# zmoon/crt1d

Measured on AMD Instinct MI355X. Metric: (column x band) solves/sec at 60 layers, higher is better.
Workload: dtype f64

## Files before the change

### crt1d_amd/_lib.py

```python

import ctypes
import os

_HERE = os.path.dirname(os.path.abspath(__file__))
LIB_PATH = os.environ.get("CRT1D_HIP_LIB") or os.path.join(_HERE, "libcrt1d_hip.so")

SCHEME_IDS = {"2s": 0, "4s": 1, "n79": 2, "zq": 3, "bl": 4, "g77": 5, "bf": 6, "zq_pa": 7}
F32_SCHEMES = ("2s", "4s", "n79", "zq", "bl", "g77", "bf", "zq_pa")
TAU_D_METHODS = {"quad": 0, "9sky": 1}
NQ_TAU, NQ_G4, NQ_9SKY = 96, 32, 9
NQ = NQ_TAU + NQ_G4 + NQ_9SKY

FLAG_SKIP_PRECOMPUTE = 1
FLAG_PRECOMPUTE_ONLY = 2
FLAG_DIRECT_STORES = 4

MAX_LEVEL_SELECT = 64

CRT_OK = 0
CRT_ERR_BAD_ARG = -1
CRT_ERR_WORKSPACE = -2
CRT_ERR_UNSUPPORTED = -3
CRT_ERR_LAUNCH = -4
CRT_ERR_SHAPE = -5

_vp = ctypes.c_void_p


class CrtColumns(ctypes.Structure):
    _fields_ = [
        ("ncol", ctypes.c_int32),
        ("nz", ctypes.c_int32),
        ("psi", _vp),
        ("lai", _vp),
        ("mla", _vp),
        ("g_kind", _vp),
        ("g_param", _vp),
        ("g_at_psi", _vp),
        ("g_table", _vp),
    ]


class CrtBands(ctypes.Structure):
    _fields_ = [
        ("nb", ctypes.c_int32),
        ("col_stride", ctypes.c_int64),
        ("I_dr0", _vp),
        ("I_df0", _vp),
        ("leaf_r", _vp),
        ("leaf_t", _vp),
        ("soil_r", _vp),
    ]


class CrtSunSeries(ctypes.Structure):

    _fields_ = [
        ("nt", ctypes.c_int32),
        ("psi", _vp),
        ("g_at_psi", _vp),
        ("col_stride", ctypes.c_int64),
        ("I_dr0", _vp),
        ("I_df0", _vp),
    ]


class CrtSunSeriesF32(CrtSunSeries):
    """crt_sun_series_f32: the layout of crt_sun_series with float I_dr0 / I_df0 behind the pointers (crt_hip_levels_series_f32)."""


NTUNE = 16

TUNE_TILE_LDS = 0
TUNE_TILE_T = 1
TUNE_TILE_FLAGS = 2
TUNE_CLOSED_STORE_WAVES = 3
TUNE_CLOSED_PIPE_T = 4
TUNE_PACK = 5
TUNE_PACK_COMPUTE_WAVES = 6
TUNE_TRI_M = 8
TUNE_TRI_T = 9
TUNE_TRI_FAMILY = 10
TUNE_TRI_STORE_WAVES = 11
TUNE_MIN_TILE_NB = 12
TUNE_FLAT_FLUSH = 13
TUNE_K0_SEPARATE = 15
TILE_FLAG_SYNC_BARRIERS = 1
TILE_FLAG_GENERIC_FLUSH = 2
TILE_FLAG_NO_PIPELINE = 4
TILE_FLAG_NO_GENERIC_PIPELINE = 8
TILE_FLAG_FOUR_PAIR_STORE = 16
PACK_OFF = 1
PACK_FORCE = 2
TRI_FAMILY_NO_PIPELINE = 1
TRI_FAMILY_DOUBLE_BUFFERED = 2
TRI_FAMILY_REG_STAGED = 3
TRI_FAMILY_GENERIC_PIPELINE = 4
TRI_FAMILY_ZQPA_TWO_KERNEL = 1
TRI_FAMILY_ZQPA_PIPE = 5
TRI_FAMILY_ZQPA_PIPE2_DB = 6
TRI_FAMILY_ZQPA_PIPE2_RS = 7
FLAT_FLUSH_OFF = 1
FLAT_FLUSH_PART_LINE = 2
FLAT_FLUSH_WHOLE_LINE = 3


class CrtOptions(ctypes.Structure):
    _fields_ = [("mu_s", ctypes.c_double), ("tau_d_method", ctypes.c_int32), ("flags", ctypes.c_int32), ("tune", ctypes.c_int32 * NTUNE)]


def set_tune(opts, tune):
    for k in tune:
        if not isinstance(k, int) or not 0 <= k < NTUNE:
            raise ValueError(f"unknown crt_options.tune key {k!r}: keys are the TUNE_* constants, 0 .. {NTUNE - 1}")
    for k in range(NTUNE):
        opts.tune[k] = int(tune.get(k, 0))
    return opts


class CrtOutputs(ctypes.Structure):
    _fields_ = [(k, _vp) for k in ("I_dr", "I_df_d", "I_df_u", "F", "x0", "x1", "x2")]


class CrtBandsumOut(ctypes.Structure):

    _fields_ = [(k, _vp) for k in ("aI", "aI_sl", "aI_sh", "totals", "aI_dr", "I_dr", "I_df_d", "I_df_u", "F", "I_d")]


ABI_VERSION = 3


def _signatures():
    P = ctypes.POINTER
    i, i32, i64, sz, dbl, ok = ctypes.c_int, ctypes.c_int32, ctypes.c_int64, ctypes.c_size_t, ctypes.c_double, ctypes.c_int
    cols, bands, opts, outs, sums = P(CrtColumns), P(CrtBands), P(CrtOptions), P(CrtOutputs), P(CrtBandsumOut)
    solve = [cols, bands, opts, outs, _vp, sz, _vp]
    t = {
        "crt_hip_abi_version": (i, None),
        "crt_hip_strerror": (ctypes.c_char_p, [i]),
        "crt_hip_workspace_bytes": (sz, [i, i32, i32]),
        "crt_hip_workspace_bytes_nb": (sz, [i, i32, i32, i32]),
        "crt_hip_series_workspace_bytes": (sz, [i, i32, i32, i32, i32]),
        "crt_hip_levels_series_workspace_bytes": (sz, [i, i32, i32, i32]),
        "crt_hip_quad_nodes": (ok, [dbl, P(dbl)]),
        "crt_hip_integrated_series_f64": (ok, [i, cols, bands, P(CrtSunSeries), opts, _vp, i32, sums, _vp, sz, _vp]),
    }
    for suffix, sun_t in (("f64", CrtSunSeries), ("f32", CrtSunSeriesF32)):
        t[f"crt_hip_solve_{suffix}"] = (ok, [i] + solve)
        for s in SCHEME_IDS if suffix == "f64" else F32_SCHEMES:
            t[f"crt_hip_{s}_{suffix}"] = (ok, solve)
        t[f"crt_hip_absorb_{suffix}"] = (ok, [cols, bands, _vp, _vp, _vp, P(_vp), _vp, _vp, _vp])
        t[f"crt_hip_absorb_bandsum_{suffix}"] = (ok, [cols, bands, _vp, _vp, _vp, _vp, i32, _vp, _vp, _vp, _vp, _vp])
        t[f"crt_hip_absorb_bandsum2_{suffix}"] = (ok, [cols, bands, _vp, _vp, _vp, _vp, i32, sums, _vp])
        t[f"crt_hip_integrated_{suffix}"] = (ok, [i, cols, bands, opts, _vp, i32, _vp, _vp, _vp, _vp, _vp, sz, _vp])
        t[f"crt_hip_integrated2_{suffix}"] = (ok, [i, cols, bands, opts, _vp, i32, sums, _vp, sz, _vp])
        t[f"crt_hip_levels_{suffix}"] = (ok, [i, cols, bands, opts, P(i32), i32, outs, _vp, sz, _vp])
        t[f"crt_hip_levels_series_{suffix}"] = (ok, [i, cols, bands, P(sun_t), opts, P(i32), i32, outs, _vp, sz, _vp])
    t.update({
        "crt_hip_bandsum_finish_f64": (ok, [cols, i32, sums, _vp]),
        "crt_hip_band_reduce_f64": (ok, [_vp, i64, i32, _vp, i32, _vp, _vp]),
        "crt_hip_tau_d_f64": (ok, [_vp, _vp, i64, i32, _vp, _vp]),
        "crt_hip_smear_tuv_f64": (ok, [_vp, i64, i32, _vp, i32, _vp, i32, _vp, _vp]),
        "crt_hip_lai_beta_f64": (ok, [_vp, _vp, _vp, i32, i32, _vp, _vp, _vp, _vp]),
        "crt_hip_buffer_alloc_set": (ok, [i32, P(sz), P(_vp)]),
        "crt_hip_buffer_alloc": (ok, [sz, P(_vp)]),
        "crt_hip_buffer_free": (ok, [_vp]),
        "crt_hip_buffer_trim": (ok, []),
        "crt_hip_buffer_set_retain": (ok, [sz]),
        "crt_hip_buffer_describe": (ok, [_vp, ctypes.c_char_p, sz]),
        "crt_hip_buffer_stats": (ok, [P(i64)]),
        "crt_hip_last_kernel": (ctypes.c_char_p, []),
        "crt_hip_probe_fill_f64": (ok, [_vp, sz, dbl, _vp]),
        "crt_hip_probe_copy_f64": (ok, [_vp, _vp, sz, _vp]),
        "crt_hip_probe_store_set_f64": (ok, [P(_vp), i32, i64, i64, i32, dbl, _vp]),
# ... 61 lines not shown
```

### crt1d_amd/csrc/crt_internal.hpp

```cpp
#pragma once
#include <hip/hip_runtime.h>
#include <stddef.h>
#include <stdint.h>

#include "crt1d_hip.h"

namespace crt {

enum RecScalar {
  S_KB = 0,
  S_MU = 1,
  S_G = 2,
  S_MUBAR = 3,
  S_GINT1 = 4,
  S_GINT2 = 5,
  S_DLM = 6,
  S_TAUI = 7,
  S_TPSI = 8,
  S_COS2 = 9,
  S_LT = 10,
  S_INVMU = 11,
  S_UNIF = 12,
  S_DL = 13,
  S_M = 14,
// ... 258 lines not shown
  double* aI_dr;
  double* L_dr;
  double* L_dn;
  double* L_up;
  double* L_F;
  double* L_Id;
};

template <int CTRL>
__device__ inline double dpp_add(double v) {
  const int lo = __builtin_amdgcn_update_dpp(0, __double2loint(v), CTRL, 0xf, 0xf, false);
  const int hi = __builtin_amdgcn_update_dpp(0, __double2hiint(v), CTRL, 0xf, 0xf, false);
  return v + __hiloint2double(hi, lo);
}
__device__ inline double row_sum16(double v) {
  v = dpp_add<0xB1>(v);
  v = dpp_add<0x4E>(v);
  v = dpp_add<0x141>(v);
  v = dpp_add<0x140>(v);
  return v;
}
template <int CTRL, int ROW_MASK>
__device__ inline double dpp_add_rows(double v) {
  const int lo = __builtin_amdgcn_update_dpp(0, __double2loint(v), CTRL, ROW_MASK, 0xf, false);
  const int hi = __builtin_amdgcn_update_dpp(0, __double2hiint(v), CTRL, ROW_MASK, 0xf, false);
  return v + __hiloint2double(hi, lo);
}
__device__ inline double wave_sum_lane63(double v) {
  v = row_sum16(v);
  v = dpp_add_rows<0x142, 0xA>(v);
  v = dpp_add_rows<0x143, 0xC>(v);
  return v;
}
__device__ inline double swap_add32(double x, double y) {
  const auto lo = __builtin_amdgcn_permlane32_swap(__double2loint(x), __double2loint(y), false, false);
  const auto hi = __builtin_amdgcn_permlane32_swap(__double2hiint(x), __double2hiint(y), false, false);
  return __hiloint2double(hi[0], lo[0]) + __hiloint2double(hi[1], lo[1]);
}
__device__ inline double swap_add16(double x, double y) {
  const auto lo = __builtin_amdgcn_permlane16_swap(__double2loint(x), __double2loint(y), false, false);
  const auto hi = __builtin_amdgcn_permlane16_swap(__double2hiint(x), __double2hiint(y), false, false);
  return __hiloint2double(hi[0], lo[0]) + __hiloint2double(hi[1], lo[1]);
}
__device__ inline double wave_sum4(double a, double b, double c, double d) {
  return row_sum16(swap_add16(swap_add32(a, b), swap_add32(c, d)));
}
__device__ inline int wave_sum4_slot(int row) { return ((row & 1) << 1) | (row >> 1); }
template <int N>
__device__ inline void wave_sum_store(const double (&v)[N], double* dst, int nvalid, int lane) {
  const int slot = wave_sum4_slot(lane >> 4);
#pragma unroll
  for (int j = 0; j < (N + 3) / 4; ++j) {
    const double z = wave_sum4(v[4 * j], 4 * j + 1 < N ? v[4 * j + 1] : 0.0, 4 * j + 2 < N ? v[4 * j + 2] : 0.0, 4 * j + 3 < N ? v[4 * j + 3] : 0.0);
    const int idx = 4 * j + slot;
    if ((lane & 15) == 0 && idx < nvalid) dst[idx] = z;
  }
}

__device__ inline double half_sum2(double x, double y) { return row_sum16(swap_add16(x, y)); }
template <int N>
__device__ inline void half_sum_store(const double (&v)[N], double* dst, int nvalid, int lane) {
  const int which = (lane >> 4) & 1;
#pragma unroll
  for (int j = 0; j < (N + 1) / 2; ++j) {
    const double z = half_sum2(v[2 * j], 2 * j + 1 < N ? v[2 * j + 1] : 0.0);
    const int idx = 2 * j + which;
    if ((lane & 15) == 0 && idx < nvalid) dst[idx] = z;
  }
}

__device__ inline double wave_sum_all(double v) {
#pragma unroll
  for (int off = 32; off > 0; off >>= 1) v += __shfl_xor(v, off, 64);
  return v;
}

struct IntLds {
  double* part;
  double* ends;
  double* pdr;
  double* lev;
  double* pi0;
};
__device__ inline IntLds int_lds_carve(double* base, int nz, int nwave, bool prof) {
  IntLds L;
  L.part = base;
  L.ends = L.part + (size_t)nz * nwave * INT_MAXG;
  L.pdr = L.ends + (size_t)2 * nwave * 2 * INT_MAXG;
  L.lev = L.pdr + (size_t)nwave * INT_MAXG;
  L.pi0 = L.lev + (prof ? (size_t)nz * nwave * 2 * INT_MAXG : 0);
  return L;
}

template <bool ROWS, bool PROF = false>
__device__ inline void int_accumulate(const IntLds& L, int nwave, int wave, int lane, int nz, int j, int ng, const double (&w)[INT_MAXG],
                                      bool active, double idr, double dn, double up) {
  if constexpr (!ROWS) {
    if constexpr (PROF) {
      const int g2 = wave_sum4_slot(lane >> 4);
      const double dd = active ? dn : 0.0, uu = active ? up : 0.0;
      const double zd = wave_sum4(w[0] * dd, w[1] * dd, w[2] * dd, w[3] * dd);
      const double zu = wave_sum4(w[0] * uu, w[1] * uu, w[2] * uu, w[3] * uu);
      if ((lane & 15) == 0 && g2 < ng) {
        L.lev[((j * nwave + wave) * 2 + 0) * INT_MAXG + g2] = zd;
        L.lev[((j * nwave + wave) * 2 + 1) * INT_MAXG + g2] = zu;
      }
    }
    const int g = wave_sum4_slot(lane >> 4);
    const bool writer = (lane & 15) == 0 && g < ng;
    const double net = active ? idr + dn - up : 0.0;
    const double z = wave_sum4(w[0] * net, w[1] * net, w[2] * net, w[3] * net);
    if (writer) L.part[(j * nwave + wave) * INT_MAXG + g] = z;
    if (j == 0 || j == nz - 1) {
      const int e = j == 0 ? 0 : 1;
      const double dd = active ? idr + dn : 0.0, uu = active ? up : 0.0;
      const double z0 = wave_sum4(w[0] * dd, w[1] * dd, w[2] * dd, w[3] * dd);
      const double z1 = wave_sum4(w[0] * uu, w[1] * uu, w[2] * uu, w[3] * uu);
      if (writer) {
        L.ends[((e * nwave + wave) * 2 + 0) * INT_MAXG + g] = z0;
        L.ends[((e * nwave + wave) * 2 + 1) * INT_MAXG + g] = z1;
      }
    }
    return;
  }
  const int nslot = ROWS ? nwave * 4 : nwave;
  const int slot = ROWS ? wave * 4 + (lane >> 4) : wave;
  const bool writer = ROWS ? (lane & 15) == 0 : lane == 63;
  auto red = [](double v) { return ROWS ? row_sum16(v) : wave_sum_lane63(v); };
  const double net = active ? idr + dn - up : 0.0;
#pragma unroll
  for (int g = 0; g < INT_MAXG; ++g)
    if (g < ng) {
      const double t = red(w[g] * net);
      if (writer) L.part[(j * nslot + slot) * INT_MAXG + g] = t;
    }
  if (j == 0 || j == nz - 1) {
    const int e = j == 0 ? 0 : 1;
#pragma unroll
    for (int g = 0; g < INT_MAXG; ++g)
      if (g < ng) {
        const double t0 = red(active ? w[g] * (idr + dn) : 0.0);
        const double t1 = red(active ? w[g] * up : 0.0);
        if (writer) {
          L.ends[((e * nslot + slot) * 2 + 0) * INT_MAXG + g] = t0;
          L.ends[((e * nslot + slot) * 2 + 1) * INT_MAXG + g] = t1;
        }
      }
  }
}

template <bool ROWS, bool PROF = false>
__device__ inline void int_finish(const IntLds& L, const IntArgs& ia, int nwave, int nz, int c, double Kb, double invmu = 0.0) {
  __syncthreads();
  if constexpr (PROF) {
    const int ngp = ia.ngroup;
    for (int i = threadIdx.x; i < nz * ngp; i += blockDim.x) {
      const int j = i / ngp, g = i - j * ngp;
      double p0 = 0.0, sD = 0.0, sU = 0.0;
      for (int wv = 0; wv < nwave; ++wv) {
        p0 += L.pi0[wv * INT_MAXG + g];
        sD += L.lev[((j * nwave + wv) * 2 + 0) * INT_MAXG + g];
        sU += L.lev[((j * nwave + wv) * 2 + 1) * INT_MAXG + g];
      }
      const double sR = exp(-Kb * ia.lai[(long long)c * nz + j]) * p0;
      const long long o = ((long long)c * nz + j) * ngp + g;
      ia.L_dr[o] = sR;
      ia.L_dn[o] = sD;
      ia.L_up[o] = sU;
      ia.L_F[o] = sR * invmu + 2 * (sU + sD);
      ia.L_Id[o] = sR + sD;
    }
  }
  const int ng = ia.ngroup, nrow = ROWS ? nwave * 4 : nwave;
  const double* lai = ia.lai + (long long)c * nz;
  for (int i = threadIdx.x; i < (nz - 1) * ng; i += blockDim.x) {
    const int k = i / ng, g = i - k * ng;
    double p0 = 0.0, p1 = 0.0, pd = 0.0;
    for (int r = 0; r < nrow; ++r) {
      p0 += L.part[(k * nrow + r) * INT_MAXG + g];
      p1 += L.part[((k + 1) * nrow + r) * INT_MAXG + g];
    }
    for (int wv = 0; wv < nwave; ++wv) pd += L.pdr[wv * INT_MAXG + g];
    const double dl = lai[k] - lai[k + 1];
    const double fsl = exp(-Kb * ((lai[k] + lai[k + 1]) / 2));
    const double adr = (1 - exp(-Kb * dl)) * exp(-Kb * lai[k + 1]) * pd;
    const double a = p1 - p0;
    const double adf = a - adr;
    const long long o = ((long long)c * (nz - 1) + k) * ng + g;
    ia.aI[o] = a;
    ia.aI_sl[o] = adf * fsl + adr;
    ia.aI_sh[o] = adf * (1 - fsl);
    if constexpr (PROF) ia.aI_dr[o] = adr;
  }
  if (ia.totals) {
    for (int i = threadIdx.x; i < ng * 4; i += blockDim.x) {
      const int g = i >> 2, q = i & 3;
      const int e = q < 2 ? 1 : 0, which = q & 1;
      double t = 0.0;
      for (int r = 0; r < nrow; ++r) t += L.ends[((e * nrow + r) * 2 + which) * INT_MAXG + g];
      ia.totals[((long long)c * ng + g) * 4 + q] = t;
    }
  }
}

__host__ __device__ inline size_t int_lds_doubles(int nz, int nwave, bool rows = false, bool prof = false) {
  const size_t nslot = rows ? (size_t)nwave * 4 : (size_t)nwave;
  return (size_t)nz * nslot * INT_MAXG + 2 * nslot * 2 * INT_MAXG + (size_t)nwave * INT_MAXG +
         (prof ? (size_t)nz * nwave * 2 * INT_MAXG + (size_t)nwave * INT_MAXG : 0);
}

constexpr int SUN_HDR = 8;
constexpr int SER_XI = 104;
__host__ __device__ inline int sun_nvec(int scheme) {
  switch (scheme) {
    case CRT_SCHEME_N79: return 5;
    case CRT_SCHEME_ZQ_PA: return 2;
    default: return 1;
  }
}
__host__ __device__ inline int sun_vec_slot(int scheme, int sv) {
  switch (scheme) {
    case CRT_SCHEME_N79: return sv < 2 ? sv : sv + 1;
    case CRT_SCHEME_ZQ: return 0;
    case CRT_SCHEME_ZQ_PA: return sv;
    default: return 1;
  }
}
__host__ __device__ inline int sun_len(int scheme, int nz) { return SUN_HDR + sun_nvec(scheme) * nz; }
__host__ __device__ inline int can_len(int scheme, int nz) { return rec_len(scheme, nz) + (scheme == CRT_SCHEME_ZQ_PA ? SER_XI : 0); }
__device__ inline int sun_hdr_slot(int i) { return i == 0 ? S_KB : i == 1 ? S_MU : i == 2 ? S_G : i == 3 ? S_INVMU : S_TPSI; }

__host__ __device__ inline int rec_vec_sun(int scheme, int vec) {
  switch (scheme) {
    case CRT_SCHEME_N79: return vec < 2 ? vec : (vec >= 3 && vec <= 5) ? vec - 1 : -1;
    case CRT_SCHEME_ZQ: return vec == 0 ? 0 : -1;
    case CRT_SCHEME_ZQ_PA: return vec < 2 ? vec : -1;
    default: return vec == 1 ? 0 : -1;
  }
}

struct SeriesArgs {
  int nt, scheme, nz;
  int canlen, sunlen;
  const double* can;
  const double* sun;
  long long col_stride;
  const void* I_dr0;
  const void* I_df0;
};

int launch_colpre_series(const ColArgs& ca, int nt, double* sun, hipStream_t s);

inline dim3 series_grid(int ncol, int nt) {
  const unsigned gy = nt < 65535 ? (unsigned)nt : 65535u;
  return dim3((unsigned)ncol, gy, (unsigned)((nt + (long long)gy - 1) / gy));
}

template <class K, class... Args>
inline int launch_kernel(K kern, dim3 grid, int nthr, size_t sh, hipStream_t s, Args... args) {
  if (sh > 64 * 1024 &&
      hipFuncSetAttribute(reinterpret_cast<const void*>(kern), hipFuncAttributeMaxDynamicSharedMemorySize, (int)sh) != hipSuccess)
    return (int)CRT_ERR_LAUNCH;
  hipLaunchKernelGGL(kern, grid, dim3(nthr), sh, s, args...);
  return hipGetLastError() == hipSuccess ? (int)CRT_OK : (int)CRT_ERR_LAUNCH;
}

__device__ __forceinline__ void series_assemble(const SeriesArgs& sr, int reclen, int c, long long v, double* lds) {
  const int tid = threadIdx.x, nthr = blockDim.x, nz = sr.nz;
  {
    const double* can = sr.can + (long long)c * sr.canlen;
    const double* sun = sr.sun + v * sr.sunlen;
    if (tid < REC_HDR) {
      int si = -1;
#pragma unroll
      for (int i = 0; i < 5; ++i)
        if (sun_hdr_slot(i) == tid) si = i;
      lds[tid] = si >= 0 ? sun[si] : can[tid];
    }
    const int nvec = (reclen - REC_HDR) / nz;
    for (int vec = 0; vec < nvec; ++vec) {
      const int sv = rec_vec_sun(sr.scheme, vec);
      const double* src = sv >= 0 ? sun + SUN_HDR + sv * nz : can + REC_HDR + vec * nz;
      for (int j = tid; j < nz; j += nthr) lds[REC_HDR + vec * nz + j] = src[j];
    }
  }
  __syncthreads();
}

template <class Body>
__device__ __forceinline__ void series_step(const SolveArgs& a, const IntArgs& ia, const SeriesArgs& sr, double* lds, Body body) {
  const int c = blockIdx.x, nz = sr.nz, ng = ia.ngroup;
// ... 100 lines not shown
```

### crt1d_amd/csrc/solve_closed.hip

```cpp
#include <algorithm>
#include <type_traits>

#include "col_record.hpp"

namespace crt {
namespace {

constexpr double PI = 3.14159265358979323846;

struct BandIn {
  double I_dr0, I_df0, r, t, s;
};

template <int MODE>
__device__ __forceinline__ bool exact_here(bool unif, int j) {
  if constexpr (MODE == 0) return true;
  if constexpr (MODE == 1) return exact_level(j);
  return !unif || exact_level(j);
}

template <typename TIO>
__device__ inline BandIn load_band(const SolveArgs& a, int c, int b, bool need_soil) {
  const long long i = (long long)c * a.col_stride + b;
  BandIn in;
// ... 905 lines not shown
  int st;
  if (fused) {
    if (nthr <= 256) st = go(k_tile<S, TIO, 256, true>);
    else if (nthr <= 512) st = go(k_tile<S, TIO, 512, true>);
    else st = go(k_tile<S, TIO, 1024, true>);
  } else {
    if (nthr <= 256) st = go(k_tile<S, TIO, 256, false>);
    else if (nthr <= 512) st = go(k_tile<S, TIO, 512, false>);
    else st = go(k_tile<S, TIO, 1024, false>);
  }
  done = st == CRT_OK;
  return st;
}

template <class S, typename TIO, int VEC, bool USE_LDS>
int launch_direct_v(const SolveArgs& a, size_t lds_bytes, hipStream_t s) {
  const long long items = (long long)a.ncol * (a.nb / VEC);
  const long long nblk = (items + DBLOCK - 1) / DBLOCK;
  if (nblk > 0x7fffffffLL) return CRT_ERR_UNSUPPORTED;
  hipLaunchKernelGGL((k_direct<S, TIO, VEC, USE_LDS>), dim3((unsigned)nblk), dim3(DBLOCK), USE_LDS ? lds_bytes : 0, s, a);
  if (hipGetLastError() != hipSuccess) return CRT_ERR_LAUNCH;
  note_kernel("k_direct<%s,%s> VEC=%d", S::NAME, sizeof(TIO) == 8 ? "f64" : "f32", VEC);
  return CRT_OK;
}

template <class S, typename TIO>
int launch_scheme(const SolveArgs& a, hipStream_t s, int force, const ColArgs* k0) {
  if (force != 1) {
    bool done;
    int st = launch_tile<S, TIO>(a, s, done, k0);
    if (st != CRT_OK || done) return st;
  }
  if (const int st = k0_before(k0, s)) return st;
  bool vec2 = (a.nb % 2 == 0) && (a.col_stride % 2 == 0);
  for (int i = 0; i < S::NARR && vec2; ++i)
    if (reinterpret_cast<uintptr_t>(a.o[i]) & (2 * sizeof(TIO) - 1)) vec2 = false;
  const int nbv = a.nb / (vec2 ? 2 : 1);
  const long long cols_per_block = (DBLOCK - 1) / nbv + 2;
  const size_t lds_bytes = (size_t)cols_per_block * a.reclen * sizeof(double);
  const bool use_lds = lds_bytes <= (size_t)MAX_DIRECT_LDS;
  if (vec2)
    return use_lds ? launch_direct_v<S, TIO, 2, true>(a, lds_bytes, s) : launch_direct_v<S, TIO, 2, false>(a, lds_bytes, s);
  return use_lds ? launch_direct_v<S, TIO, 1, true>(a, lds_bytes, s) : launch_direct_v<S, TIO, 1, false>(a, lds_bytes, s);
}

template <class S>
int launch_io(const SolveArgs& a, hipStream_t s, int force, const ColArgs* k0) {
  return a.f32 ? launch_scheme<S, float>(a, s, force, k0) : launch_scheme<S, double>(a, s, force, k0);
}

template <class S, typename TIO, bool PROF>
__device__ __forceinline__ void int_body(const SolveArgs& a, const IntArgs& ia, int rec_dbl, double* lds) {
  const int nb = a.nb, nz = a.nz, ng = ia.ngroup;
  const int tid = threadIdx.x, nthr = blockDim.x, lane = tid & 63, wave = tid >> 6, nwave = nthr >> 6;
  const int c = blockIdx.x;
  const double* rec = lds;
  const IntLds L = int_lds_carve(lds + rec_dbl, nz, nwave, PROF);
  const bool active = tid < nb;
  const int b = active ? tid : 0;
  const BandIn in = load_band<TIO>(a, c, b, S::SOIL);
  S st;
  st.init(rec, in, a);
  double w[INT_MAXG];
#pragma unroll
  for (int g = 0; g < INT_MAXG; ++g) w[g] = (g < ng && active) ? ia.band_w[(long long)g * nb + b] : 0.0;
#pragma unroll
  for (int g = 0; g < INT_MAXG; ++g)
    if (g < ng) {
      const double t = wave_sum_all(w[g] * (1 - (in.r + in.t)) * in.I_dr0);
      if (lane == 0) L.pdr[wave * INT_MAXG + g] = t;
      if constexpr (PROF) {
        const double t0 = wave_sum_all(w[g] * in.I_dr0);
        if (lane == 0) L.pi0[wave * INT_MAXG + g] = t0;
      }
    }
  for (int j = 0; j < nz; ++j) {
    double val[S::NARR];
    st.level(j, rec, nz, val);
    int_accumulate<false, PROF>(L, nwave, wave, lane, nz, j, ng, w, active, val[0], val[1], val[2]);
  }
  int_finish<false, PROF>(L, ia, nwave, nz, c, rec[S_KB], rec[S_INVMU]);
}

template <class S, typename TIO, int MAXT, bool PROF>
__global__ __launch_bounds__(MAXT) void k_int(SolveArgs a, IntArgs ia, int rec_dbl) {
  extern __shared__ double lds[];
  {
    const double* src = a.ws + (long long)blockIdx.x * a.reclen;
    for (int i = threadIdx.x; i < a.reclen; i += blockDim.x) lds[i] = src[i];
  }
  __syncthreads();
  int_body<S, TIO, PROF>(a, ia, rec_dbl, lds);
}

template <class S, int MAXT, bool PROF>
__global__ __launch_bounds__(MAXT) void k_int_series(SolveArgs a, IntArgs ia, SeriesArgs sr, int rec_dbl) {
  extern __shared__ double lds[];
  series_step(a, ia, sr, lds, [&](const SolveArgs& at, const IntArgs& it) { int_body<S, double, PROF>(at, it, rec_dbl, lds); });
}

template <class S, typename TIO>
int launch_int(const SolveArgs& a, const IntArgs& ia, hipStream_t s, const SeriesArgs* sr) {
  if (a.nb > 1024) return CRT_ERR_UNSUPPORTED;
  const int nthr = ((a.nb + 63) / 64) * 64;
  const int rec_dbl = (a.reclen + 1) & ~1;
  const bool prof = ia.L_dr != nullptr;
  const size_t sh = (rec_dbl + int_lds_doubles(a.nz, nthr / 64, false, prof)) * sizeof(double);
  if (sh > 160 * 1024) return CRT_ERR_UNSUPPORTED;
  if (sr) {
    if constexpr (sizeof(TIO) == 8) {
      auto gos = [&](auto kern) {
        const int st = launch_kernel(kern, series_grid(a.ncol, sr->nt), nthr, sh, s, a, ia, *sr, rec_dbl);
        if (st == CRT_OK) note_kernel("k_colpre<canopy> + k_colsun + k_int_series<%s>%s nt=%d", S::NAME, prof ? " + level profiles" : " wave totals", sr->nt);
        return st;
      };
      if (prof) return nthr <= 256 ? gos(k_int_series<S, 256, true>) : nthr <= 512 ? gos(k_int_series<S, 512, true>) : gos(k_int_series<S, 1024, true>);
      return nthr <= 256 ? gos(k_int_series<S, 256, false>) : nthr <= 512 ? gos(k_int_series<S, 512, false>) : gos(k_int_series<S, 1024, false>);
    }
    return CRT_ERR_UNSUPPORTED;
  }
  auto go = [&](auto kern) {
    if (const int st = launch_kernel(kern, dim3(a.ncol), nthr, sh, s, a, ia, rec_dbl)) return st;
    note_kernel("k_int<%s>%s%s", S::NAME, sizeof(TIO) == 8 ? "" : " f32", prof ? " + level profiles" : " wave totals");
    return (int)CRT_OK;
  };
  if (prof) {
    if (nthr <= 256) return go(k_int<S, TIO, 256, true>);
    if (nthr <= 512) return go(k_int<S, TIO, 512, true>);
    return go(k_int<S, TIO, 1024, true>);
  }
  if (nthr <= 256) return go(k_int<S, TIO, 256, false>);
  if (nthr <= 512) return go(k_int<S, TIO, 512, false>);
  return go(k_int<S, TIO, 1024, false>);
}

template <class S>
int launch_int_io(const SolveArgs& a, const IntArgs& ia, hipStream_t s, const SeriesArgs* sr) {
  return a.f32 ? launch_int<S, float>(a, ia, s, sr) : launch_int<S, double>(a, ia, s, sr);
}

template <class S, typename TIO>
__device__ __forceinline__ void lev_body(const SolveArgs& a, const LevArgs& la, int per, const double* rec, int slice, long long oshift) {
  const int c = blockIdx.x, nz = a.nz, nb = a.nb;
  const int b = slice * per + threadIdx.x;
  if ((int)threadIdx.x >= per || b >= nb) return;
  S st;
  st.init(rec, load_band<TIO>(a, c, b, S::SOIL), a);
  const bool unif = rec[S_UNIF] != 0.0;
  const int nsel = la.nsel;
  int next = 0;
  for (int r = 0; r < nsel; ++r) {
    const int j = la.lev[r];
    const int j0 = max(unif ? (j & ~7) : j, next);
    double val[S::NARR];
    for (int jj = j0; jj <= j; ++jj) st.level(jj, rec, nz, val);
    next = j + 1;
    const long long o = ((long long)c * nsel + r) * nb + b + oshift;
#pragma unroll
    for (int q = 0; q < 4; ++q)
      if (la.o[q]) __builtin_nontemporal_store((TIO)val[q], outp<TIO>(la.o[q]) + o);
  }
}

template <class S, typename TIO, int MAXT, bool USE_LDS>
__global__ __launch_bounds__(MAXT) void k_lev(SolveArgs a, LevArgs la, int per) {
  extern __shared__ double lds[];
  const double* rec = a.ws + (long long)blockIdx.x * a.reclen;
  if constexpr (USE_LDS) {
    for (int i = threadIdx.x; i < a.reclen; i += blockDim.x) lds[i] = rec[i];
    __syncthreads();
    rec = lds;
  }
  lev_body<S, TIO>(a, la, per, rec, blockIdx.y, 0);
}

template <class S, typename TIO, int MAXT>
__global__ __launch_bounds__(MAXT) void k_lev_series(SolveArgs a, LevArgs la, SeriesArgs sr, int per, int nslice) {
  extern __shared__ double lds[];
  series_lev_step<TIO>(a, la, sr, nslice, lds,
                       [&](const SolveArgs& at, int slice, long long oshift) { lev_body<S, TIO>(at, la, per, lds, slice, oshift); });
}

template <class S, typename TIO>
int launch_lev(const SolveArgs& a, const LevArgs& la, hipStream_t s, const SeriesArgs* sr, bool probe) {
  const LevSlices ls = lev_slices(a.nb, 1024);
  if (ls.nslice > 65535) return CRT_ERR_UNSUPPORTED;
  const size_t sh = (size_t)a.reclen * sizeof(double);
  const bool use_lds = sh <= 160 * 1024;
  if (sr) {
    dim3 grid;
    if (!use_lds || !lev_series_grid(a.ncol, sr->nt, ls.nslice, &grid)) return CRT_ERR_UNSUPPORTED;
    if (probe) return CRT_OK;
    auto gos = [&](auto kern) {
      const int st = launch_kernel(kern, grid, ls.nthr, sh, s, a, la, *sr, ls.per, ls.nslice);
      if (st == CRT_OK)
        note_kernel("k_colpre<canopy> + k_colsun + k_lev_series<%s>%s nsel=%d slice=%d nt=%d", S::NAME, sizeof(TIO) == 8 ? "" : " f32", la.nsel,
                    ls.per, sr->nt);
      return st;
    };
    return ls.nthr <= 256 ? gos(k_lev_series<S, TIO, 256>) : ls.nthr <= 512 ? gos(k_lev_series<S, TIO, 512>) : gos(k_lev_series<S, TIO, 1024>);
  }
  if (probe) return CRT_OK;
  auto go = [&](auto kern) {
    const size_t shk = use_lds ? sh : 0;
    if (const int st = launch_kernel(kern, dim3(a.ncol, ls.nslice), ls.nthr, shk, s, a, la, ls.per)) return st;
    note_kernel("k_lev<%s>%s nsel=%d slice=%d%s", S::NAME, sizeof(TIO) == 8 ? "" : " f32", la.nsel, ls.per,
                use_lds ? "" : " record in HBM");
    return (int)CRT_OK;
// ... 58 lines not shown
```

### include/crt1d_hip.h

```cpp
#ifndef CRT1D_HIP_H
#define CRT1D_HIP_H

#include <stddef.h>
#include <stdint.h>

#ifdef __cplusplus
extern "C" {
#endif

#define CRT_ABI_VERSION 3

enum crt_g_kind {
  CRT_G_HORIZONTAL = 0,
  CRT_G_SPHERICAL = 1,
  CRT_G_VERTICAL = 2,
  CRT_G_ELLIPSOIDAL = 3,
  CRT_G_ELLIPSOIDAL_APPROX = 4,
  CRT_G_ELLIPSOIDAL_APPROX_BONAN = 5,
  CRT_G_TABLE = 6
};

#define CRT_NQ_TAU 96
#define CRT_NQ_G4 32
#define CRT_NQ_9SKY 9
#define CRT_NQ (CRT_NQ_TAU + CRT_NQ_G4 + CRT_NQ_9SKY)

enum crt_scheme {
  CRT_SCHEME_2S = 0, CRT_SCHEME_4S = 1, CRT_SCHEME_N79 = 2, CRT_SCHEME_ZQ = 3,
  CRT_SCHEME_BL = 4, CRT_SCHEME_G77 = 5, CRT_SCHEME_BF = 6, CRT_SCHEME_ZQ_PA = 7, CRT_NUM_SCHEMES = 8
};

enum crt_tau_d_method { CRT_TAU_D_QUAD = 0, CRT_TAU_D_9SKY = 1 };

enum crt_status {
  CRT_OK = 0,
  CRT_ERR_BAD_ARG = -1,
  CRT_ERR_WORKSPACE = -2,
  CRT_ERR_UNSUPPORTED = -3,
  CRT_ERR_LAUNCH = -4,
  CRT_ERR_SHAPE = -5
};

typedef void* crt_stream_t;

typedef struct crt_columns {
  int32_t ncol;
  int32_t nz;
  const double* psi;
  const double* lai;
  const double* mla;
  const int32_t* g_kind;
  const double* g_param;
  const double* g_at_psi;
  const double* g_table;
} crt_columns;

typedef struct crt_bands {
  int32_t nb;
  int64_t col_stride;
  const double* I_dr0;
  const double* I_df0;
  const double* leaf_r;
  const double* leaf_t;
  const double* soil_r;
} crt_bands;

#define CRT_FLAG_SKIP_PRECOMPUTE 1
#define CRT_FLAG_PRECOMPUTE_ONLY 2
#define CRT_FLAG_DIRECT_STORES 4

enum crt_tune_key {
  CRT_TUNE_TILE_LDS = 0,
  CRT_TUNE_TILE_T = 1,
  CRT_TUNE_TILE_FLAGS = 2,
  CRT_TUNE_CLOSED_STORE_WAVES = 3,
  CRT_TUNE_CLOSED_PIPE_T = 4,
  CRT_TUNE_PACK = 5,
  CRT_TUNE_PACK_COMPUTE_WAVES = 6,
  CRT_TUNE_TRI_M = 8,
  CRT_TUNE_TRI_T = 9,
  CRT_TUNE_TRI_FAMILY = 10,
  CRT_TUNE_TRI_STORE_WAVES = 11,
  CRT_TUNE_MIN_TILE_NB = 12,
  CRT_TUNE_FLAT_FLUSH = 13,
  CRT_TUNE_K0_SEPARATE = 15
};
#define CRT_NTUNE 16

enum crt_tune_tile_flag {
  CRT_TILE_FLAG_SYNC_BARRIERS = 1,
  CRT_TILE_FLAG_GENERIC_FLUSH = 2,
  CRT_TILE_FLAG_NO_PIPELINE = 4,
  CRT_TILE_FLAG_NO_GENERIC_PIPELINE = 8,
  CRT_TILE_FLAG_FOUR_PAIR_STORE = 16
};

enum crt_tune_pack {
  CRT_PACK_OFF = 1,
  CRT_PACK_FORCE = 2
};

enum crt_tune_tri_family {
  CRT_TRI_FAMILY_NO_PIPELINE = 1,
  CRT_TRI_FAMILY_DOUBLE_BUFFERED = 2,
  CRT_TRI_FAMILY_REG_STAGED = 3,
  CRT_TRI_FAMILY_GENERIC_PIPELINE = 4,
  CRT_TRI_FAMILY_ZQPA_TWO_KERNEL = 1,
  CRT_TRI_FAMILY_ZQPA_PIPE = 5,
  CRT_TRI_FAMILY_ZQPA_PIPE2_DB = 6,
  CRT_TRI_FAMILY_ZQPA_PIPE2_RS = 7
};

enum crt_tune_flat_flush {
  CRT_FLAT_FLUSH_OFF = 1,
  CRT_FLAT_FLUSH_PART_LINE = 2,
  CRT_FLAT_FLUSH_WHOLE_LINE = 3
};

typedef struct crt_options {
  double mu_s;
  int32_t tau_d_method;
  int32_t flags;
  int32_t tune[CRT_NTUNE];
} crt_options;

typedef struct crt_outputs {
  double* I_dr;
  double* I_df_d;
  double* I_df_u;
  double* F;
  double* x0;
  double* x1;
  double* x2;
} crt_outputs;

typedef struct crt_bands_f32 {
  int32_t nb;
  int64_t col_stride;
  const float* I_dr0;
  const float* I_df0;
  const float* leaf_r;
  const float* leaf_t;
  const float* soil_r;
} crt_bands_f32;

typedef struct crt_outputs_f32 {
  float* I_dr;
  float* I_df_d;
  float* I_df_u;
  float* F;
  float* x0;
  float* x1;
  float* x2;
} crt_outputs_f32;

int crt_hip_abi_version(void);
const char* crt_hip_strerror(int status);

size_t crt_hip_workspace_bytes(int scheme, int32_t ncol, int32_t nz);

size_t crt_hip_workspace_bytes_nb(int scheme, int32_t ncol, int32_t nz, int32_t nb);

int crt_hip_quad_nodes(double mu_s, double* psi_nodes);

int crt_hip_solve_f64(int scheme, const crt_columns* cols, const crt_bands* bands, const crt_options* opts,
                      const crt_outputs* out, void* workspace, size_t workspace_bytes, crt_stream_t stream);
int crt_hip_2s_f64(const crt_columns*, const crt_bands*, const crt_options*, const crt_outputs*, void*, size_t, crt_stream_t);
int crt_hip_4s_f64(const crt_columns*, const crt_bands*, const crt_options*, const crt_outputs*, void*, size_t, crt_stream_t);
int crt_hip_n79_f64(const crt_columns*, const crt_bands*, const crt_options*, const crt_outputs*, void*, size_t, crt_stream_t);
int crt_hip_zq_f64(const crt_columns*, const crt_bands*, const crt_options*, const crt_outputs*, void*, size_t, crt_stream_t);
int crt_hip_bl_f64(const crt_columns*, const crt_bands*, const crt_options*, const crt_outputs*, void*, size_t, crt_stream_t);
int crt_hip_g77_f64(const crt_columns*, const crt_bands*, const crt_options*, const crt_outputs*, void*, size_t, crt_stream_t);
int crt_hip_bf_f64(const crt_columns*, const crt_bands*, const crt_options*, const crt_outputs*, void*, size_t, crt_stream_t);
int crt_hip_zq_pa_f64(const crt_columns*, const crt_bands*, const crt_options*, const crt_outputs*, void*, size_t, crt_stream_t);

int crt_hip_solve_f32(int scheme, const crt_columns* cols, const crt_bands_f32* bands, const crt_options* opts,
                      const crt_outputs_f32* out, void* workspace, size_t workspace_bytes, crt_stream_t stream);
// ... 116 lines not shown
```

Before: 3.534 billion.

## Add dedicated reduce wave for band-integrated level sums with double-buffered LDS tiles

The integrated kernel gets a new form in which compute waves write per-level band values into a double-buffered LDS tile of four levels. A separate extra wave reduces the tile against band weights while the compute waves move on to the next tile, replacing the per-wave cross-lane reductions at every level. The form is on by default when it fits in LDS and adds a wave, extra LDS and a barrier per tile. Tune flags can force either form.

```diff
diff --git a/crt1d_amd/_lib.py b/crt1d_amd/_lib.py
--- a/crt1d_amd/_lib.py
+++ b/crt1d_amd/_lib.py
@@ -90,6 +90,8 @@
 TILE_FLAG_NO_PIPELINE = 4
 TILE_FLAG_NO_GENERIC_PIPELINE = 8
 TILE_FLAG_FOUR_PAIR_STORE = 16
+INT_FORM_IN_WAVE = 32
+INT_FORM_REDUCE_WAVE = 64
 PACK_OFF = 1
 PACK_FORCE = 2
 TRI_FAMILY_NO_PIPELINE = 1
diff --git a/crt1d_amd/csrc/crt_internal.hpp b/crt1d_amd/csrc/crt_internal.hpp
--- a/crt1d_amd/csrc/crt_internal.hpp
+++ b/crt1d_amd/csrc/crt_internal.hpp
@@ -364,14 +364,27 @@
   double* lev;
   double* pi0;
 };
-__device__ inline IntLds int_lds_carve(double* base, int nz, int nwave, bool prof) {
+__device__ inline IntLds int_lds_carve(double* base, int nz, int nwave, bool prof, int nlev = 0) {
   IntLds L;
+  if (nlev == 0) nlev = nwave;
   L.part = base;
-  L.ends = L.part + (size_t)nz * nwave * INT_MAXG;
+  L.ends = L.part + (size_t)nz * nlev * INT_MAXG;
   L.pdr = L.ends + (size_t)2 * nwave * 2 * INT_MAXG;
   L.lev = L.pdr + (size_t)nwave * INT_MAXG;
-  L.pi0 = L.lev + (prof ? (size_t)nz * nwave * 2 * INT_MAXG : 0);
+  L.pi0 = L.lev + (prof ? (size_t)nz * nlev * 2 * INT_MAXG : 0);
   return L;
+}
+
+__device__ inline void int_ends(const IntLds& L, int nwave, int wave, int lane, int e, int ng, const double (&w)[INT_MAXG], bool active,
+                                double idr, double dn, double up) {
+  const int g = wave_sum4_slot(lane >> 4);
+  const double dd = active ? idr + dn : 0.0, uu = active ? up : 0.0;
+  const double z0 = wave_sum4(w[0] * dd, w[1] * dd, w[2] * dd, w[3] * dd);
+  const double z1 = wave_sum4(w[0] * uu, w[1] * uu, w[2] * uu, w[3] * uu);
+  if ((lane & 15) == 0 && g < ng) {
+    L.ends[((e * nwave + wave) * 2 + 0) * INT_MAXG + g] = z0;
+    L.ends[((e * nwave + wave) * 2 + 1) * INT_MAXG + g] = z1;
+  }
 }
 
 template <bool ROWS, bool PROF = false>
@@ -393,16 +406,7 @@
     const double net = active ? idr + dn - up : 0.0;
     const double z = wave_sum4(w[0] * net, w[1] * net, w[2] * net, w[3] * net);
     if (writer) L.part[(j * nwave + wave) * INT_MAXG + g] = z;
-    if (j == 0 || j == nz - 1) {
-      const int e = j == 0 ? 0 : 1;
-      const double dd = active ? idr + dn : 0.0, uu = active ? up : 0.0;
-      const double z0 = wave_sum4(w[0] * dd, w[1] * dd, w[2] * dd, w[3] * dd);
-      const double z1 = wave_sum4(w[0] * uu, w[1] * uu, w[2] * uu, w[3] * uu);
-      if (writer) {
-        L.ends[((e * nwave + wave) * 2 + 0) * INT_MAXG + g] = z0;
-        L.ends[((e * nwave + wave) * 2 + 1) * INT_MAXG + g] = z1;
-      }
-    }
+    if (j == 0 || j == nz - 1) int_ends(L, nwave, wave, lane, j == 0 ? 0 : 1, ng, w, active, idr, dn, up);
     return;
   }
   const int nslot = ROWS ? nwave * 4 : nwave;
@@ -432,17 +436,18 @@
 }
 
 template <bool ROWS, bool PROF = false>
-__device__ inline void int_finish(const IntLds& L, const IntArgs& ia, int nwave, int nz, int c, double Kb, double invmu = 0.0) {
+__device__ inline void int_finish(const IntLds& L, const IntArgs& ia, int nwave, int nz, int c, double Kb, double invmu = 0.0, int nlev = 0) {
   __syncthreads();
+  const int nlw = nlev ? nlev : nwave;
   if constexpr (PROF) {
     const int ngp = ia.ngroup;
     for (int i = threadIdx.x; i < nz * ngp; i += blockDim.x) {
       const int j = i / ngp, g = i - j * ngp;
       double p0 = 0.0, sD = 0.0, sU = 0.0;
-      for (int wv = 0; wv < nwave; ++wv) {
-        p0 += L.pi0[wv * INT_MAXG + g];
-        sD += L.lev[((j * nwave + wv) * 2 + 0) * INT_MAXG + g];
-        sU += L.lev[((j * nwave + wv) * 2 + 1) * INT_MAXG + g];
+      for (int wv = 0; wv < nwave; ++wv) p0 += L.pi0[wv * INT_MAXG + g];
+      for (int wv = 0; wv < nlw; ++wv) {
+        sD += L.lev[((j * nlw + wv) * 2 + 0) * INT_MAXG + g];
+        sU += L.lev[((j * nlw + wv) * 2 + 1) * INT_MAXG + g];
       }
       const double sR = exp(-Kb * ia.lai[(long long)c * nz + j]) * p0;
       const long long o = ((long long)c * nz + j) * ngp + g;
@@ -458,9 +463,10 @@
   for (int i = threadIdx.x; i < (nz - 1) * ng; i += blockDim.x) {
     const int k = i / ng, g = i - k * ng;
     double p0 = 0.0, p1 = 0.0, pd = 0.0;
-    for (int r = 0; r < nrow; ++r) {
-      p0 += L.part[(k * nrow + r) * INT_MAXG + g];
-      p1 += L.part[((k + 1) * nrow + r) * INT_MAXG + g];
+    const int npart = nlev ? nlev : nrow;
+    for (int r = 0; r < npart; ++r) {
+      p0 += L.part[(k * npart + r) * INT_MAXG + g];
+      p1 += L.part[((k + 1) * npart + r) * INT_MAXG + g];
     }
     for (int wv = 0; wv < nwave; ++wv) pd += L.pdr[wv * INT_MAXG + g];
     const double dl = lai[k] - lai[k + 1];
@@ -485,10 +491,52 @@
   }
 }
 
-__host__ __device__ inline size_t int_lds_doubles(int nz, int nwave, bool rows = false, bool prof = false) {
+__host__ __device__ inline size_t int_lds_doubles(int nz, int nwave, bool rows = false, bool prof = false, int nlev = 0) {
   const size_t nslot = rows ? (size_t)nwave * 4 : (size_t)nwave;
-  return (size_t)nz * nslot * INT_MAXG + 2 * nslot * 2 * INT_MAXG + (size_t)nwave * INT_MAXG +
-         (prof ? (size_t)nz * nwave * 2 * INT_MAXG + (size_t)nwave * INT_MAXG : 0);
+  const size_t npart = nlev ? (size_t)nlev : nslot, nlw = nlev ? (size_t)nlev : (size_t)nwave;
+  return (size_t)nz * npart * INT_MAXG + 2 * nslot * 2 * INT_MAXG + (size_t)nwave * INT_MAXG +
+         (prof ? (size_t)nz * nlw * 2 * INT_MAXG + (size_t)nwave * INT_MAXG : 0);
+}
+
+constexpr int INT_RT = 4;
+__host__ __device__ inline int int_tile_nbp(int nb) { return (nb + 7) & ~7; }
+__host__ __device__ inline int int_tile_stride(int nb) {
+  const int nbp = int_tile_nbp(nb);
+  return nbp % 16 == 8 ? nbp : nbp + 8;
+}
+__host__ __device__ inline size_t int_tile_doubles(int nb, bool prof) {
+  return (size_t)int_tile_stride(nb) * (INT_MAXG + 2 * INT_RT * (prof ? 3 : 1));
+}
+
+template <bool PROF>
+__device__ inline void int_tile_reduce(const IntLds& L, const double* xt, const double* wl, int ls, int nbp, int lane, int j0, int nz, int ng) {
+  constexpr int Q = PROF ? 3 : 1;
+  const int jj = lane >> 4, g = (lane >> 2) & 3, s = lane & 3;
+  const double* x = xt + (size_t)jj * Q * ls + 2 * s;
+  const double* wg = wl + (size_t)g * ls + 2 * s;
+  double e[Q], o[Q];
+#pragma unroll
+  for (int q = 0; q < Q; ++q) e[q] = o[q] = 0.0;
+#pragma unroll 4
+  for (int i = 0; i < nbp; i += 8) {
+    const double2 wv = *reinterpret_cast<const double2*>(wg + i);
+#pragma unroll
+    for (int q = 0; q < Q; ++q) {
+      const double2 xv = *reinterpret_cast<const double2*>(x + q * ls + i);
+      e[q] = fma(wv.x, xv.x, e[q]);
+      o[q] = fma(wv.y, xv.y, o[q]);
+    }
+  }
+  const int j = j0 + jj;
+  const bool writer = s == 0 && g < ng && j < nz;
+#pragma unroll
+  for (int q = 0; q < Q; ++q) {
+    const double z = dpp_add<0x4E>(dpp_add<0xB1>(e[q] + o[q]));
+    if (writer) {
+      if (q == 0) L.part[j * INT_MAXG + g] = z;
+      else L.lev[(j * 2 + (q - 1)) * INT_MAXG + g] = z;
+    }
+  }
 }
 
 constexpr int SUN_HDR = 8;
diff --git a/crt1d_amd/csrc/solve_closed.hip b/crt1d_amd/csrc/solve_closed.hip
--- a/crt1d_amd/csrc/solve_closed.hip
+++ b/crt1d_amd/csrc/solve_closed.hip
@@ -1011,48 +1011,145 @@
   int_finish<false, PROF>(L, ia, nwave, nz, c, rec[S_KB], rec[S_INVMU]);
 }
 
-template <class S, typename TIO, int MAXT, bool PROF>
-__global__ __launch_bounds__(MAXT) void k_int(SolveArgs a, IntArgs ia, int rec_dbl) {
+template <class S, typename TIO, bool PROF>
+__device__ __forceinline__ void int_body_rw(const SolveArgs& a, const IntArgs& ia, int rec_dbl, double* lds, int ncw) {
+  constexpr int Q = PROF ? 3 : 1;
+  const int nb = a.nb, nz = a.nz, ng = ia.ngroup;
+  const int tid = threadIdx.x, nthr = blockDim.x, lane = tid & 63, wave = tid >> 6;
+  const int c = blockIdx.x;
+  const double* rec = lds;
+  const IntLds L = int_lds_carve(lds + rec_dbl, nz, ncw, PROF, 1);
+  const int ls = int_tile_stride(nb), nbp = int_tile_nbp(nb);
+  double* wl = lds + rec_dbl + int_lds_doubles(nz, ncw, false, PROF, 1);
+  double* tile = wl + INT_MAXG * ls;
+  const bool compute = wave < ncw, reduce = wave == (nthr > ncw * 64 ? ncw : 0);
+  const bool active = tid < nb, put = tid < nbp;
+  for (int i = tid; i < INT_MAXG * ls; i += nthr) {
+    const int g = i / ls, bb = i - g * ls;
+    wl[i] = (g < ng && bb < nb) ? ia.band_w[(long long)g * nb + bb] : 0.0;
+  }
+  S st;
+  double w[INT_MAXG];
+  if (compute) {
+    const int b = active ? tid : 0;
+    const BandIn in = load_band<TIO>(a, c, b, S::SOIL);
+    st.init(rec, in, a);
+#pragma unroll
+    for (int g = 0; g < INT_MAXG; ++g) w[g] = (g < ng && active) ? ia.band_w[(long long)g * nb + b] : 0.0;
+#pragma unroll
+    for (int g = 0; g < INT_MAXG; ++g)
+      if (g < ng) {
+        const double t = wave_sum_all(w[g] * (1 - (in.r + in.t)) * in.I_dr0);
+        if (lane == 0) L.pdr[wave * INT_MAXG + g] = t;
+        if constexpr (PROF) {
+          const double t0 = wave_sum_all(w[g] * in.I_dr0);
+          if (lane == 0) L.pi0[wave * INT_MAXG + g] = t0;
+        }
+      }
+  }
+  const int ntile = (nz + INT_RT - 1) / INT_RT;
+  for (int t = 0; t <= ntile; ++t) {
+    if (compute && t < ntile) {
+      double* x = tile + (size_t)(t & 1) * INT_RT * Q * ls + tid;
+      const int j1 = min(nz, (t + 1) * INT_RT);
+      for (int j = t * INT_RT; j < j1; ++j, x += Q * ls) {
+        double val[S::NARR];
+        st.level(j, rec, nz, val);
+        if (put) {
+          x[0] = active ? val[0] + val[1] - val[2] : 0.0;
+          if constexpr (PROF) {
+            x[ls] = active ? val[1] : 0.0;
+            x[2 * ls] = active ? val[2] : 0.0;
+          }
+        }
+        if (j == 0 || j == nz - 1) int_ends(L, ncw, wave, lane, j == 0 ? 0 : 1, ng, w, active, val[0], val[1], val[2]);
+      }
+    }
+    if (reduce && t > 0)
+      int_tile_reduce<PROF>(L, tile + (size_t)((t - 1) & 1) * INT_RT * Q * ls, wl, ls, nbp, lane, (t - 1) * INT_RT, nz, ng);
+    if (t < ntile) lds_barrier();
+  }
+  int_finish<false, PROF>(L, ia, ncw, nz, c, rec[S_KB], rec[S_INVMU], 1);
+}
+
+template <class S, typename TIO, int MAXT, bool PROF, bool RW = false>
+__global__ __launch_bounds__(MAXT) void k_int(SolveArgs a, IntArgs ia, int rec_dbl, int ncw) {
   extern __shared__ double lds[];
   {
     const double* src = a.ws + (long long)blockIdx.x * a.reclen;
     for (int i = threadIdx.x; i < a.reclen; i += blockDim.x) lds[i] = src[i];
   }
   __syncthreads();
-  int_body<S, TIO, PROF>(a, ia, rec_dbl, lds);
-}
-
-template <class S, int MAXT, bool PROF>
-__global__ __launch_bounds__(MAXT) void k_int_series(SolveArgs a, IntArgs ia, SeriesArgs sr, int rec_dbl) {
+  if constexpr (RW) int_body_rw<S, TIO, PROF>(a, ia, rec_dbl, lds, ncw);
+  else int_body<S, TIO, PROF>(a, ia, rec_dbl, lds);
+}
+
+template <class S, int MAXT, bool PROF, bool RW = false>
+__global__ __launch_bounds__(MAXT) void k_int_series(SolveArgs a, IntArgs ia, SeriesArgs sr, int rec_dbl, int ncw) {
   extern __shared__ double lds[];
-  series_step(a, ia, sr, lds, [&](const SolveArgs& at, const IntArgs& it) { int_body<S, double, PROF>(at, it, rec_dbl, lds); });
+  series_step(a, ia, sr, lds, [&](const SolveArgs& at, const IntArgs& it) {
+    if constexpr (RW) int_body_rw<S, double, PROF>(at, it, rec_dbl, lds, ncw);
+    else int_body<S, double, PROF>(at, it, rec_dbl, lds);
+  });
+}
+
+inline bool int_rw_default(int nb, bool prof) { return true; }
+struct IntForm {
+  bool rw;
+  int ncw, nthr;
+  size_t sh;
+};
+inline IntForm int_form(const SolveArgs& a, bool prof) {
+  IntForm f;
+  f.ncw = (a.nb + 63) / 64;
+  const int rec_dbl = (a.reclen + 1) & ~1;
+  const size_t sh_rw = (rec_dbl + int_lds_doubles(a.nz, f.ncw, false, prof, 1) + int_tile_doubles(a.nb, prof)) * sizeof(double);
+  const int flags = a.tune.tile_flags;
+  const bool fits = sh_rw <= 160 * 1024;
+  const bool want = (flags & CRT_INT_FORM_REDUCE_WAVE) ? true : int_rw_default(a.nb, prof);
+  f.rw = fits && want && !(flags & CRT_INT_FORM_IN_WAVE);
+  f.nthr = f.rw ? min(1024, f.ncw * 64 + 64) : f.ncw * 64;
+  f.sh = f.rw ? sh_rw : (rec_dbl + int_lds_doubles(a.nz, f.ncw, false, prof)) * sizeof(double);
+  return f;
 }
 
 template <class S, typename TIO>
 int launch_int(const SolveArgs& a, const IntArgs& ia, hipStream_t s, const SeriesArgs* sr) {
   if (a.nb > 1024) return CRT_ERR_UNSUPPORTED;
-  const int nthr = ((a.nb + 63) / 64) * 64;
   const int rec_dbl = (a.reclen + 1) & ~1;
   const bool prof = ia.L_dr != nullptr;
-  const size_t sh = (rec_dbl + int_lds_doubles(a.nz, nthr / 64, false, prof)) * sizeof(double);
+  const IntForm f = int_form(a, prof);
+  const int nthr = f.nthr, ncw = f.rw ? f.ncw : 0;
+  const size_t sh = f.sh;
   if (sh > 160 * 1024) return CRT_ERR_UNSUPPORTED;
+  char form[48];
+  if (f.rw) snprintf(form, sizeof form, " reduce_waves=%d T=%d lds=%zu", nthr > f.ncw * 64 ? 1 : 0, INT_RT, sh);
+  else snprintf(form, sizeof form, "%s", prof ? "" : " wave totals");
   if (sr) {
     if constexpr (sizeof(TIO) == 8) {
       auto gos = [&](auto kern) {
-        const int st = launch_kernel(kern, series_grid(a.ncol, sr->nt), nthr, sh, s, a, ia, *sr, rec_dbl);
-        if (st == CRT_OK) note_kernel("k_colpre<canopy> + k_colsun + k_int_series<%s>%s nt=%d", S::NAME, prof ? " + level profiles" : " wave totals", sr->nt);
+        const int st = launch_kernel(kern, series_grid(a.ncol, sr->nt), nthr, sh, s, a, ia, *sr, rec_dbl, ncw);
+        if (st == CRT_OK) note_kernel("k_colpre<canopy> + k_colsun + k_int_series<%s>%s%s nt=%d", S::NAME, prof ? " + level profiles" : "", form, sr->nt);
         return st;
       };
+      if (f.rw) {
+        if (prof) return nthr <= 512 ? gos(k_int_series<S, 512, true, true>) : gos(k_int_series<S, 1024, true, true>);
+        return nthr <= 512 ? gos(k_int_series<S, 512, false, true>) : gos(k_int_series<S, 1024, false, true>);
+      }
       if (prof) return nthr <= 256 ? gos(k_int_series<S, 256, true>) : nthr <= 512 ? gos(k_int_series<S, 512, true>) : gos(k_int_series<S, 1024, true>);
       return nthr <= 256 ? gos(k_int_series<S, 256, false>) : nthr <= 512 ? gos(k_int_series<S, 512, false>) : gos(k_int_series<S, 1024, false>);
     }
     return CRT_ERR_UNSUPPORTED;
   }
   auto go = [&](auto kern) {
-    if (const int st = launch_kernel(kern, dim3(a.ncol), nthr, sh, s, a, ia, rec_dbl)) return st;
-    note_kernel("k_int<%s>%s%s", S::NAME, sizeof(TIO) == 8 ? "" : " f32", prof ? " + level profiles" : " wave totals");
+    if (const int st = launch_kernel(kern, dim3(a.ncol), nthr, sh, s, a, ia, rec_dbl, ncw)) return st;
+    note_kernel("k_int<%s>%s%s%s", S::NAME, sizeof(TIO) == 8 ? "" : " f32", prof ? " + level profiles" : "", form);
     return (int)CRT_OK;
   };
+  if (f.rw) {
+    if (prof) return nthr <= 512 ? go(k_int<S, TIO, 512, true, true>) : go(k_int<S, TIO, 1024, true, true>);
+    return nthr <= 512 ? go(k_int<S, TIO, 512, false, true>) : go(k_int<S, TIO, 1024, false, true>);
+  }
   if (prof) {
     if (nthr <= 256) return go(k_int<S, TIO, 256, true>);
     if (nthr <= 512) return go(k_int<S, TIO, 512, true>);
diff --git a/include/crt1d_hip.h b/include/crt1d_hip.h
--- a/include/crt1d_hip.h
+++ b/include/crt1d_hip.h
@@ -93,6 +93,10 @@
   CRT_TILE_FLAG_NO_PIPELINE = 4,
   CRT_TILE_FLAG_NO_GENERIC_PIPELINE = 8,
   CRT_TILE_FLAG_FOUR_PAIR_STORE = 16
+};
+enum crt_tune_int_form {
+  CRT_INT_FORM_IN_WAVE = 32,
+  CRT_INT_FORM_REDUCE_WAVE = 64
 };
 
 enum crt_tune_pack {
```

New measurement: 3.504 billion. No clear change (-0.8%).
